# chao1224/MoleculeSDE

Hardware: AMD Instinct MI355X
Metric: molecules/sec pretrain step (SchNet+SDE VE, bs256) (higher is better)
Workload: dtype f32; 1 GPU; PCQM4Mv2-shaped pretrain step: GIN5x300 + SchNet(6x128f,51g,rc10) + EBM_node_dot_prod contrastive + SDEModel2Dto3D_02 VE; fwd+bwd+Adam; molecules_per_gpu=256, global_batch=256, parallelism=dp1

## Files before the change

moleculesde_amd/csrc/linear.hip:

```cpp
#include "msde_common.h"

typedef float f32x16 __attribute__((ext_vector_type(16)));

#define LG_BK 32
#ifndef MSDE_WGRAD_NARROW
#define MSDE_WGRAD_NARROW 7
#endif
#ifndef LG_SKIP_DEAD
#define LG_SKIP_DEAD 1
#endif
#ifndef LG_PRIO
#define LG_PRIO 2
#endif
#ifndef LG_ST
#define LG_ST 1
#endif

__device__ __forceinline__ float4 lg_ldg4(const void* p) {
#if defined(__HIP_DEVICE_COMPILE__)
  typedef float lg_v4f __attribute__((ext_vector_type(4)));
  const lg_v4f v = *(const __attribute__((address_space(1))) lg_v4f*)(p);
  return make_float4(v.x, v.y, v.z, v.w);
#else
  return *reinterpret_cast<const float4*>(p);
#endif
}
__device__ __forceinline__ float lg_ldg1(const float* p) {
#if defined(__HIP_DEVICE_COMPILE__)
  return *(const __attribute__((address_space(1))) float*)(p);
#else
  return *p;
#endif
}

#ifdef LG_PROBE
__device__ unsigned long long lg_probe[8];
#define LG_T(x) __builtin_amdgcn_sched_barrier(0); const unsigned long long x = __builtin_readcyclecounter(); __builtin_amdgcn_sched_barrier(0)
extern "C" int msde_debug_lg_probe(unsigned long long* host8, int reset) {
  if (host8 && hipMemcpyFromSymbol(host8, HIP_SYMBOL(lg_probe), sizeof(lg_probe)) != hipSuccess) return MSDE_EINVAL;
  if (reset) { unsigned long long z[8] = {0}; if (hipMemcpyToSymbol(HIP_SYMBOL(lg_probe), z, sizeof(z)) != hipSuccess) return MSDE_EINVAL; }
  return 0;
}
#else
#define LG_T(x)
#endif

template <int TM, int TN, bool A_KM, bool B_KM, bool VEC, int WGM = 2, int KS = 1>
__device__ __forceinline__ void
gemm_f32_mfma_body(const float* __restrict__ A, const float* __restrict__ B, const float* __restrict__ bias,
                   float* __restrict__ C, float* __restrict__ colsum_ws, int M, int N, int K, int lda, int ldb,
                   int ldc, int k_per_split, const int bid_x, const int bid_y, const int bid_z, float* __restrict__ As,
                   float* __restrict__ Bs, const bool edge_fast = false) {
  constexpr int WGN = KS == 4 ? 1 : 4 / WGM;
  constexpr int BM = 32 * (KS == 4 ? 1 : WGM) * TM, BN = 32 * WGN * TN;
  constexpr int BK = LG_BK * KS;
  static_assert(KS == 1 || (KS == 4 && TM == 1 && TN == 1 && WGM == 1 && A_KM && B_KM), "k-split tiles: 32 x 32, k-major operands");
  static_assert(WGM == 2 || (TM == 1 && TN == 1 && A_KM && B_KM), "side-by-side wave layouts: weight-gradient operands only");
  constexpr int LDA_S = A_KM ? (KS == 4 ? 32 : BM <= 64 ? 64 : (WGM == 2 ? BM + 4 : BM)) : BM + 1;
  constexpr int LDB_S = B_KM ? (KS == 4 ? 32 : BN <= 64 ? 64 : (WGM == 2 ? BN + 4 : BN)) : BN + 1;

  int tid_ = threadIdx.x;
  asm volatile("" : "+v"(tid_));
  const int tid = tid_, lane = tid & 63, wave = tid >> 6;
  const int lcol = lane & 31, lhalf = lane >> 5;
  const int wm = KS == 4 ? 0 : wave / WGN, wn = KS == 4 ? 0 : wave % WGN;
  const int kq = KS == 4 ? wave * LG_BK : 0;
  const int m0 = bid_y * BM, n0 = bid_x * BN;
  const int kb = bid_z * k_per_split;
  const int ke = max(min(K, kb + k_per_split), kb);

  constexpr int NA = BM * BK / 1024, NB = BN * BK / 1024;
  static_assert(NA >= 1 && NB >= 1, "tile too small for 256 threads");
  constexpr int ST = LG_ST;
  float4 rsa[ST][NA], rsb[ST][NB];

  auto ld4 = [&](const float* __restrict__ base, int row, int nrows, int ld, int col, int ncols, bool vec) -> float4 {
    bool rv = row < nrows;
    int rc = rv ? row : 0;
    const float* src = base + (size_t)rc * ld;
    float4 v;
    if (vec) {
      bool cv = col < ncols;
      v = lg_ldg4(src + (cv ? col : 0));
      if (!(rv && cv)) v = make_float4(0.f, 0.f, 0.f, 0.f);
    } else {
      float x0 = lg_ldg1(src + (col < ncols ? col : 0)), x1 = lg_ldg1(src + (col + 1 < ncols ? col + 1 : 0));
      float x2 = lg_ldg1(src + (col + 2 < ncols ? col + 2 : 0)), x3 = lg_ldg1(src + (col + 3 < ncols ? col + 3 : 0));
      v.x = (rv && col < ncols) ? x0 : 0.f;
      v.y = (rv && col + 1 < ncols) ? x1 : 0.f;
      v.z = (rv && col + 2 < ncols) ? x2 : 0.f;
      v.w = (rv && col + 3 < ncols) ? x3 : 0.f;
    }
    return v;
  };

  auto load_tile = [&](float4 (&ra)[NA], float4 (&rb)[NB], int k0) {
#pragma unroll
    for (int p = 0; p < NA; ++p) {
      int idx = p * 256 + tid;
      if (!A_KM) {
        int r = idx >> 3, kq = (idx & 7) * 4;
        ra[p] = ld4(A, m0 + r, M, lda, k0 + kq, ke, VEC);
      } else {
        int kr = idx / (BM / 4), mq = (idx % (BM / 4)) * 4;
        ra[p] = ld4(A, k0 + kr, ke, lda, m0 + mq, M, VEC);
      }
    }
#pragma unroll
    for (int p = 0; p < NB; ++p) {
      int idx = p * 256 + tid;
      if (!B_KM) {
        int r = idx >> 3, kq = (idx & 7) * 4;
        rb[p] = ld4(B, n0 + r, N, ldb, k0 + kq, ke, VEC);
      } else {
        int kr = idx / (BN / 4), nq = (idx % (BN / 4)) * 4;
        rb[p] = ld4(B, k0 + kr, ke, ldb, n0 + nq, N, VEC);
      }
    }
  };

  constexpr bool FAST = A_KM && B_KM && VEC;
  const bool interior = FAST && (edge_fast ? (M >= 4 && N >= 4) : (m0 + BM <= M && n0 + BN <= N));
  unsigned oa[NA], ob[NB];
  if (FAST) {
#pragma unroll
    for (int p = 0; p < NA; ++p) {
      const int idx = p * 256 + tid, kr = idx / (BM / 4), mq = min((idx % (BM / 4)) * 4, M - 4 - m0);
      oa[p] = (unsigned)(((long long)kr * lda + mq) * 4);
    }
#pragma unroll
    for (int p = 0; p < NB; ++p) {
      const int idx = p * 256 + tid, kr = idx / (BN / 4), nq = min((idx % (BN / 4)) * 4, N - 4 - n0);
      ob[p] = (unsigned)(((long long)kr * ldb + nq) * 4);
    }
  }
  auto load_tile_fast = [&](float4 (&ra)[NA], float4 (&rb)[NB], int k0) {
    const char* __restrict__ ab = reinterpret_cast<const char*>(A + (size_t)k0 * lda + m0);
    const char* __restrict__ bb = reinterpret_cast<const char*>(B + (size_t)k0 * ldb + n0);
#pragma unroll
    for (int p = 0; p < NA; ++p) ra[p] = lg_ldg4(ab + oa[p]);
#pragma unroll
    for (int p = 0; p < NB; ++p) rb[p] = lg_ldg4(bb + ob[p]);
  };

  auto store_tile = [&](const float4 (&ra)[NA], const float4 (&rb)[NB]) {
#pragma unroll
    for (int p = 0; p < NA; ++p) {
      int idx = p * 256 + tid;
      if (!A_KM) {
        int r = idx >> 3, kq = (idx & 7) * 4;
        As[(kq + 0) * LDA_S + r] = ra[p].x;
        As[(kq + 1) * LDA_S + r] = ra[p].y;
        As[(kq + 2) * LDA_S + r] = ra[p].z;
        As[(kq + 3) * LDA_S + r] = ra[p].w;
      } else {
        int kr = idx / (BM / 4), mq = (idx % (BM / 4)) * 4;
        *reinterpret_cast<float4*>(&As[kr * LDA_S + mq]) = ra[p];
      }
    }
#pragma unroll
    for (int p = 0; p < NB; ++p) {
      int idx = p * 256 + tid;
      if (!B_KM) {
        int r = idx >> 3, kq = (idx & 7) * 4;
        Bs[(kq + 0) * LDB_S + r] = rb[p].x;
        Bs[(kq + 1) * LDB_S + r] = rb[p].y;
        Bs[(kq + 2) * LDB_S + r] = rb[p].z;
        Bs[(kq + 3) * LDB_S + r] = rb[p].w;
      } else {
        int kr = idx / (BN / 4), nq = (idx % (BN / 4)) * 4;
        *reinterpret_cast<float4*>(&Bs[kr * LDB_S + nq]) = rb[p];
      }
    }
  };

  f32x16 acc[TM][TN];
#pragma unroll
  for (int i = 0; i < TM; ++i)
#pragma unroll
    for (int j = 0; j < TN; ++j)
#pragma unroll
      for (int r = 0; r < 16; ++r) acc[i][j][r] = 0.f;

  float csum = 0.f;

  const bool quadrant_live = !LG_SKIP_DEAD || ((m0 + wm * 32 * TM < M) && (n0 + wn * 32 * TN < N));
  bool sub_live[TM][TN];
#pragma unroll
  for (int i = 0; i < TM; ++i)
#pragma unroll
    for (int j = 0; j < TN; ++j)
      sub_live[i][j] = (m0 + (wm * TM + i) * 32 < M) && (n0 + (wn * TN + j) * 32 < N);
#ifdef LG_PROBE
  unsigned long long pt4 = 0, pacc[6] = {0, 0, 0, 0, 0, 0};
#endif
  auto compute_tile = [&]() {
    if (TM == 1 && TN == 1) {
      if (quadrant_live) {
      float af[LG_BK / 2], bf[LG_BK / 2];
#pragma unroll
      for (int kk = 0; kk < LG_BK / 2; ++kk) {
        af[kk] = As[(kq + 2 * kk + lhalf) * LDA_S + wm * 32 + lcol];
        bf[kk] = Bs[(kq + 2 * kk + lhalf) * LDB_S + wn * 32 + lcol];
      }
      __builtin_amdgcn_sched_barrier(0);
#ifdef LG_PROBE
      pt4 = __builtin_readcyclecounter();
      __builtin_amdgcn_sched_barrier(0);
#endif
      __builtin_amdgcn_s_setprio(LG_PRIO);
#pragma unroll
      for (int kk = 0; kk < LG_BK / 2; ++kk)
        acc[0][0] = __builtin_amdgcn_mfma_f32_32x32x2f32(af[kk], bf[kk], acc[0][0], 0, 0, 0);
      __builtin_amdgcn_s_setprio(0);
      }
    } else {
    __builtin_amdgcn_s_setprio(LG_PRIO);
#pragma unroll
    for (int kk = 0; kk < LG_BK / 2; ++kk) {
      float af[TM], bf[TN];
#pragma unroll
      for (int i = 0; i < TM; ++i) af[i] = As[(2 * kk + lhalf) * LDA_S + (wm * TM + i) * 32 + lcol];
#pragma unroll
      for (int j = 0; j < TN; ++j) bf[j] = Bs[(2 * kk + lhalf) * LDB_S + (wn * TN + j) * 32 + lcol];
#pragma unroll
      for (int i = 0; i < TM; ++i)
#pragma unroll
        for (int j = 0; j < TN; ++j)
          if (!LG_SKIP_DEAD || sub_live[i][j])
            acc[i][j] = __builtin_amdgcn_mfma_f32_32x32x2f32(af[i], bf[j], acc[i][j], 0, 0, 0);
    }
    __builtin_amdgcn_s_setprio(0);
    }
    if (colsum_ws != nullptr && bid_x == 0) {
      if (A_KM && (BM == 64 || WGM != 2)) {
        constexpr int CG = 256 / BM;
        const int c = tid % BM, q = tid / BM;
#pragma unroll
        for (int kr = 0; kr < BK / CG; ++kr) csum += As[(q * (BK / CG) + kr) * LDA_S + c];
      } else if (tid < BM) {
#pragma unroll 8
        for (int kr = 0; kr < LG_BK; ++kr) csum += As[kr * LDA_S + tid];
      }
    }
  };

  const int ntiles = (ke - kb + BK - 1) / BK;
  if (ntiles > 0) {
#pragma unroll
    for (int s = 0; s < ST; ++s) load_tile(rsa[s], rsb[s], kb + s * BK);
    int t = 0;
    if (FAST && interior) {
      const int nfull = (ke - kb) / BK;
      for (; t + 2 * ST <= nfull; t += ST) {
#pragma unroll
        for (int s = 0; s < ST; ++s) {
          LG_T(t0);
          __syncthreads();
          LG_T(t1);
          store_tile(rsa[s], rsb[s]);
          LG_T(t2);
          __syncthreads();
          LG_T(t3);
          load_tile_fast(rsa[s], rsb[s], kb + (t + s + ST) * BK);
          compute_tile();
          LG_T(t5);
#ifdef LG_PROBE
          pacc[0] += t1 - t0; pacc[1] += t2 - t1; pacc[2] += t3 - t2; pacc[3] += pt4 - t3; pacc[4] += t5 - pt4; pacc[5] += 1;
#endif
        }
      }
    }
    for (; t + ST <= ntiles; t += ST) {
#pragma unroll
      for (int s = 0; s < ST; ++s) {
        __syncthreads();
        store_tile(rsa[s], rsb[s]);
        __syncthreads();
        load_tile(rsa[s], rsb[s], kb + (t + s + ST) * BK);
        compute_tile();
      }
    }
    const int rem = ntiles - t;
#pragma unroll
    for (int s = 0; s < ST - 1; ++s) {
      if (s < rem) {
        __syncthreads();
        store_tile(rsa[s], rsb[s]);
        __syncthreads();
        compute_tile();
      }
    }
  }

#ifdef LG_PROBE
  if (tid == 0 && quadrant_live)
    for (int i = 0; i < 6; ++i) atomicAdd(&lg_probe[i], pacc[i]);
#endif
  float* Cz = C + (size_t)bid_z * (size_t)M * ldc;
  if (KS == 4) {
    __syncthreads();
#pragma unroll
    for (int r = 0; r < 16; ++r) As[(wave * 16 + r) * 64 + lane] = acc[0][0][r];
    __syncthreads();
    const int gn = n0 + lcol;
#pragma unroll
    for (int j = 0; j < 4; ++j) {
      const int r = 4 * wave + j;
      const float v = ((As[r * 64 + lane] + As[(16 + r) * 64 + lane]) + As[(32 + r) * 64 + lane]) + As[(48 + r) * 64 + lane];
      const int gm = m0 + (r & 3) + 8 * (r >> 2) + 4 * lhalf;
      if (gm < M && gn < N) Cz[(size_t)gm * ldc + gn] = v;
    }
  } else {
#pragma unroll
  for (int i = 0; i < TM; ++i)
#pragma unroll
    for (int j = 0; j < TN; ++j) {
      int gn = n0 + (wn * TN + j) * 32 + lcol;
      float bv = (bias != nullptr && gn < N) ? bias[gn] : 0.f;
#pragma unroll
      for (int r = 0; r < 16; ++r) {
        int gm = m0 + (wm * TM + i) * 32 + (r & 3) + 8 * (r >> 2) + 4 * lhalf;
        if (gm < M && gn < N) Cz[(size_t)gm * ldc + gn] = acc[i][j][r] + bv;
      }
    }
  }
  if (colsum_ws != nullptr && bid_x == 0) {
    if (A_KM && (BM == 64 || WGM != 2)) {
      constexpr int CG = 256 / BM;
      __syncthreads();
      Bs[tid] = csum;
      __syncthreads();
      if (tid < BM) {
        csum = Bs[tid];
#pragma unroll
        for (int q = 1; q < CG; ++q) csum += Bs[q * BM + tid];
      }
    }
    if (tid < BM && m0 + tid < M) colsum_ws[(size_t)bid_z * M + m0 + tid] = csum;
  }
}

template <int TM, int TN, bool A_KM, bool B_KM, bool VEC>
__global__ void __launch_bounds__(256)
gemm_f32_mfma_kernel(const float* __restrict__ A, const float* __restrict__ B, const float* __restrict__ bias,
                     float* __restrict__ C, float* __restrict__ colsum_ws, int M, int N, int K, int lda, int ldb,
                     int ldc, int k_per_split, const int* __restrict__ Kdev) {
  constexpr int BM = 64 * TM, BN = 64 * TN;
  constexpr int LDA_S = A_KM ? (BM == 64 ? 64 : BM + 4) : BM + 1, LDB_S = B_KM ? (BN == 64 ? 64 : BN + 4) : BN + 1;
  __shared__ __attribute__((aligned(16))) float As[LG_BK * LDA_S];
  __shared__ __attribute__((aligned(16))) float Bs[LG_BK * LDB_S];
  gemm_f32_mfma_body<TM, TN, A_KM, B_KM, VEC>(A, B, bias, C, colsum_ws, M, N, msde_true_rows(K, Kdev), lda, ldb, ldc,
                                              k_per_split, blockIdx.x, blockIdx.y, blockIdx.z, As, Bs);
}

__device__ __forceinline__ void
gemm_grouped_wgrad_body(const long long* __restrict__ probs, const int* __restrict__ prefix, int count, int total,
                          int xcd_order) {
  __shared__ __attribute__((aligned(16))) float lds[8192];
  for (int blk = blockIdx.x; blk < total; blk += gridDim.x) {
    int lo = 0, hi = count;
    while (hi - lo > 1) {
      int mid = (lo + hi) >> 1;
      if (prefix[mid] <= blk) lo = mid; else hi = mid;
    }
    const long long* e = probs + (size_t)lo * MSDE_WGRAD_ROW;
    const float* gY = reinterpret_cast<const float*>(e[0]);
    const float* X = reinterpret_cast<const float*>(e[1]);
    float* slabs = reinterpret_cast<float*>(e[2]);
    float* cs = reinterpret_cast<float*>(e[3]);
    const int M = (int)e[4], N = (int)e[5], K = (int)e[6], kps = (int)e[8], tx = (int)e[9], ty = (int)e[10];
    const int ldg = (int)e[12], ldx = (int)e[13];
    const int Mt = msde_true_rows(M, reinterpret_cast<const int*>(e[14]));
    int local = blk - prefix[lo];
    if (xcd_order) {
      const int np = prefix[lo + 1] - prefix[lo], q = np >> 3, r = np & 7, c = local & 7;
      local = c * q + min(c, r) + (local >> 3);
    }
    const int bx = local % tx, by = (local / tx) % ty, bz = local / (tx * ty);
    const int shape = (int)(e[15] >> 1);
    float* As = lds;
    float* Bs = lds + 4096;
    if ((MSDE_WGRAD_NARROW & 1) && e[11] && shape == 1)
      gemm_f32_mfma_body<1, 1, true, true, true, 1, 1>(gY, X, nullptr, slabs, cs, N, K, Mt, ldg, ldx, K, kps, bx, by, bz, As, Bs, true);
    else if ((MSDE_WGRAD_NARROW & 2) && e[11] && shape == 2)
      gemm_f32_mfma_body<1, 1, true, true, true, 4, 1>(gY, X, nullptr, slabs, cs, N, K, Mt, ldg, ldx, K, kps, bx, by, bz, As, Bs, true);
    else if ((MSDE_WGRAD_NARROW & 4) && e[11] && shape == 3)
      gemm_f32_mfma_body<1, 1, true, true, true, 1, 4>(gY, X, nullptr, slabs, cs, N, K, Mt, ldg, ldx, K, kps, bx, by, bz, As, Bs, true);
    else if (e[11])
      gemm_f32_mfma_body<1, 1, true, true, true>(gY, X, nullptr, slabs, cs, N, K, Mt, ldg, ldx, K, kps, bx, by, bz, As, Bs,
                                                 (e[15] & 1) != 0);
    else
      gemm_f32_mfma_body<1, 1, true, true, false>(gY, X, nullptr, slabs, cs, N, K, Mt, ldg, ldx, K, kps, bx, by, bz, As, Bs);
    __syncthreads();
  }
}

__global__ void __launch_bounds__(256)
gemm_grouped_wgrad_kernel(const long long* __restrict__ probs, const int* __restrict__ prefix, int count, int total,
                          int xcd_order) {
  gemm_grouped_wgrad_body(probs, prefix, count, total, xcd_order);
}
__global__ void __launch_bounds__(256) __attribute__((amdgpu_waves_per_eu(4, 4)))
gemm_grouped_wgrad_occ4_kernel(const long long* __restrict__ probs, const int* __restrict__ prefix, int count, int total,
                               int xcd_order) {
  gemm_grouped_wgrad_body(probs, prefix, count, total, xcd_order);
}

#define RS_LANES 16
__global__ void __launch_bounds__(256)
reduce_slabs_kernel(const float* __restrict__ slabs, int splits, size_t n, float* __restrict__ out,
                    const float* __restrict__ cs, size_t nb, float* __restrict__ outb) {
  __shared__ float part[RS_LANES][16];
  const int ox = threadIdx.x & 15, ly = threadIdx.x >> 4;
  size_t total = n + (cs ? nb : 0);
  for (size_t base = (size_t)blockIdx.x * 16; base < total; base += (size_t)gridDim.x * 16) {
    size_t i = base + ox;
    float acc = 0.f;
    if (i < total) {
      const float* src = i < n ? slabs + i : cs + (i - n);
      size_t stride = i < n ? n : nb;
      for (int z = ly; z < splits; z += RS_LANES) acc += src[(size_t)z * stride];
    }
    part[ly][ox] = acc;
    __syncthreads();
    if (ly == 0 && i < total) {
      float r = part[0][ox];
#pragma unroll
      for (int l = 1; l < RS_LANES; ++l) r += part[l][ox];
      if (i < n) out[i] = r; else outb[i - n] = r;
    }
    __syncthreads();
  }
}

int msde_reduce_slabs(const float* slabs, int splits, size_t n, float* out, const float* cs, size_t nb, float* outb,
                      hipStream_t st) {
  size_t total = n + (cs ? nb : 0);
  int blocks = (int)((total + 15) / 16);
  if (blocks > 4096) blocks = 4096;
  if (blocks < 1) blocks = 1;
  MSDE_LAUNCH(reduce_slabs_kernel, dim3(blocks), dim3(256), 0, st, slabs, splits, n, out, cs, nb, outb);
  MSDE_CHECK_LAUNCH();
  return 0;
}

static inline bool aligned16(const void* p) { return (reinterpret_cast<uintptr_t>(p) & 15) == 0; }

template <int TM, int TN, bool A_KM, bool B_KM>
static void launch_cfg(bool vec, dim3 grid, hipStream_t st, const float* A, const float* B, const float* bias, float* C,
                       float* colsum_ws, int M, int N, int K, int lda, int ldb, int ldc, int k_per_split, const int* kdev) {
  if (vec)
    MSDE_LAUNCH((gemm_f32_mfma_kernel<TM, TN, A_KM, B_KM, true>), grid, dim3(256), 0, st, A, B, bias, C, colsum_ws, M, N,
                K, lda, ldb, ldc, k_per_split, kdev);
  else
    MSDE_LAUNCH((gemm_f32_mfma_kernel<TM, TN, A_KM, B_KM, false>), grid, dim3(256), 0, st, A, B, bias, C, colsum_ws, M,
                N, K, lda, ldb, ldc, k_per_split, kdev);
}

template <bool A_KM, bool B_KM>
static int launch_gemm(const float* A, const float* B, const float* bias, float* C, float* colsum_ws, int M, int N,
                       int K, int lda, int ldb, int ldc, int splits, int k_per_split, bool big, hipStream_t st,
                       const int* kdev = nullptr) {
  bool vec = aligned16(A) && aligned16(B) && (lda % 4 == 0) && (ldb % 4 == 0) && (k_per_split % 4 == 0);
  vec = vec && ((A_KM ? M : K) % 4 == 0) && ((B_KM ? N : K) % 4 == 0);
  int tm, tn;
  if (big) {
    tm = M > 64 ? 2 : 1;
    tn = N > 64 ? 2 : 1;
  } else {
    long t22 = (long)((M + 127) / 128) * ((N + 127) / 128);
    long t21 = (long)((M + 127) / 128) * ((N + 63) / 64);
    if (t22 >= 384) { tm = 2; tn = 2; }
    else if (t21 >= 256) { tm = 2; tn = 1; }
    else { tm = 1; tn = 1; }
  }
  dim3 grid((N + 64 * tn - 1) / (64 * tn), (M + 64 * tm - 1) / (64 * tm), splits);
#define LG_ARGS vec, grid, st, A, B, bias, C, colsum_ws, M, N, K, lda, ldb, ldc, k_per_split, kdev
  if (tm == 2 && tn == 2) launch_cfg<2, 2, A_KM, B_KM>(LG_ARGS);
  else if (tm == 2 && tn == 1) launch_cfg<2, 1, A_KM, B_KM>(LG_ARGS);
  else if (tm == 1 && tn == 2) launch_cfg<1, 2, A_KM, B_KM>(LG_ARGS);
  else launch_cfg<1, 1, A_KM, B_KM>(LG_ARGS);
#undef LG_ARGS
  hipError_t e = hipGetLastError();
  return e == hipSuccess ? 0 : (int)e;
}

__global__ void __launch_bounds__(256) zero_words_kernel(uint32_t* __restrict__ p, size_t n) {
  for (size_t i = (size_t)blockIdx.x * 256 + threadIdx.x; i < n; i += (size_t)gridDim.x * 256) p[i] = 0u;
}
__global__ void __launch_bounds__(256) zero_words4_kernel(uint4* __restrict__ p, size_t n4) {
  for (size_t i = (size_t)blockIdx.x * 256 + threadIdx.x; i < n4; i += (size_t)gridDim.x * 256) p[i] = make_uint4(0u, 0u, 0u, 0u);
}

int msde_zero_words(void* p, size_t n_words, hipStream_t st) {
  if (n_words == 0) return 0;
  if (!p || (reinterpret_cast<uintptr_t>(p) & 3)) return MSDE_EINVAL;
  if ((reinterpret_cast<uintptr_t>(p) & 15) == 0 && n_words % 4 == 0) {
    size_t n4 = n_words / 4, wg = (n4 + 255) / 256;
    MSDE_LAUNCH(zero_words4_kernel, dim3((unsigned)(wg < 4096 ? wg : 4096)), dim3(256), 0, st, reinterpret_cast<uint4*>(p), n4);
  } else {
    size_t wg = (n_words + 255) / 256;
    MSDE_LAUNCH(zero_words_kernel, dim3((unsigned)(wg < 4096 ? wg : 4096)), dim3(256), 0, st, reinterpret_cast<uint32_t*>(p), n_words);
  }
  MSDE_CHECK_LAUNCH();
  return 0;
}

extern "C" int msde_linear_fwd(const float* X, const float* W, const float* bias, int M, int N, int K, float* Y,
                               void* stream) {
  if (M < 0 || N <= 0 || K <= 0 || !X || !W || !Y) return MSDE_EINVAL;
  if (M == 0) return 0;
  return launch_gemm<false, false>(X, W, bias, Y, nullptr, M, N, K, K, K, N, 1, (K + 31) / 32 * 32, false,
                                    as_stream(stream));
}

extern "C" int msde_linear_bwd_x(const float* gY, const float* W, int M, int N, int K, float* gX, void* stream) {
  if (M < 0 || N <= 0 || K <= 0 || !gY || !W || !gX) return MSDE_EINVAL;
  if (M == 0) return 0;
  return launch_gemm<false, true>(gY, W, nullptr, gX, nullptr, M, K, N, N, K, K, 1, (N + 31) / 32 * 32, false,
                                   as_stream(stream));
}

static inline bool wgrad_big(int M, int N, int K) {
  return false;
}
static inline void wgrad_split_for(int M, int N, int K, int target, int* splits, int* k_per_split);
static inline void wgrad_split(int M, int N, int K, int* splits, int* k_per_split) {
  const int target = 512;
  wgrad_split_for(M, N, K, target, splits, k_per_split);
}
#ifndef MSDE_WGRAD_TARGET
#define MSDE_WGRAD_TARGET 64
#endif
#ifndef MSDE_WGRAD_MIN_ROWS
#define MSDE_WGRAD_MIN_ROWS 256
#endif
#ifndef MSDE_WGRAD_TARGET_KS
#define MSDE_WGRAD_TARGET_KS 64
#endif
static inline void wgrad_split_batched(int M, int N, int K, int* splits, int* k_per_split) {
  const int target = (N <= 32 && K <= 32 && (MSDE_WGRAD_NARROW & 4)) ? MSDE_WGRAD_TARGET_KS : MSDE_WGRAD_TARGET;
  wgrad_split_for(M, N, K, target, splits, k_per_split);
}
static inline void wgrad_split_for(int M, int N, int K, int target, int* splits, int* k_per_split) {
  bool big = wgrad_big(M, N, K);
  int tw_n = (big && N > 64) ? 128 : 64, tw_k = (big && K > 64) ? 128 : 64;
  long tiles = (long)((N + tw_n - 1) / tw_n) * ((K + tw_k - 1) / tw_k);
  long want = (target + tiles - 1) / tiles;
  long maxs = (M + MSDE_WGRAD_MIN_ROWS - 1) / MSDE_WGRAD_MIN_ROWS;
  if (maxs < 1) maxs = 1;
  if (want > maxs) want = maxs;
  if (want > 512) want = 512;
  if (want < 1) want = 1;
  int kps = (int)(((M + want - 1) / want + LG_BK - 1) / LG_BK * LG_BK);
  if (kps < LG_BK) kps = LG_BK;
  *k_per_split = kps;
  *splits = M > 0 ? (M + kps - 1) / kps : 1;
}

static inline bool wgrad_group_plan(int M, int N, int K, int* splits, int* k_per_split) {
  wgrad_split_batched(M, N, K, splits, k_per_split);
  return false;
}

extern "C" long long msde_linear_bwd_w_workspace_bytes(int M, int N, int K) {
  int splits, kps;
  wgrad_split(M, N, K, &splits, &kps);
  return (long long)splits * ((long long)N * K + N) * (long long)sizeof(float);
}

__global__ void __launch_bounds__(256)
reduce_slabs_multi_kernel(const long long* __restrict__ rows, const int* __restrict__ prefix, int count) {
  __shared__ float4 part[256];
  int lo = 0, hi = count;
  while (hi - lo > 1) {
    int mid = (lo + hi) >> 1;
    if (prefix[mid] <= (int)blockIdx.x) lo = mid; else hi = mid;
  }
  const long long* e = rows + (size_t)lo * 8;
  const float* slabs = reinterpret_cast<const float*>(e[0]);
  const int splits = (int)e[1];
  const size_t n = (size_t)e[2];
  float* out = reinterpret_cast<float*>(e[3]);
  const size_t row_len = (size_t)e[4], slab_ld = (size_t)e[5], out_ld = (size_t)e[6], sstride = (size_t)e[7];
  const int LY = splits >= MSDE_REDUCE_LONG ? 16 : 4, OXN = 256 / LY;
  const int ox = threadIdx.x % OXN, ly = threadIdx.x / OXN;
  const size_t i = (size_t)(blockIdx.x - prefix[lo]) * (4 * OXN) + 4 * ox;
  const bool flat = row_len == n;
  const bool vec = (n % 4 == 0) && ((reinterpret_cast<uintptr_t>(slabs) | reinterpret_cast<uintptr_t>(out)) & 15) == 0 &&
                   (flat ? sstride % 4 == 0 : ((row_len | slab_ld | out_ld | sstride) % 4 == 0));
  size_t so[4], oo[4];
#pragma unroll
  for (int q = 0; q < 4; ++q) {
    const size_t j = i + q;
    if (flat) { so[q] = j; oo[q] = j; }
    else { const size_t r = j / row_len, c = j - r * row_len; so[q] = r * slab_ld + c; oo[q] = r * out_ld + c; }
  }
  float4 acc = make_float4(0.f, 0.f, 0.f, 0.f);
  if (i < n) {
    if (vec) {
      const float* base = slabs + so[0];
      int z = ly;
      for (; z + 3 * LY < splits; z += 4 * LY) {
        float4 a = *reinterpret_cast<const float4*>(base + (size_t)z * sstride);
        float4 b = *reinterpret_cast<const float4*>(base + (size_t)(z + LY) * sstride);
        float4 c = *reinterpret_cast<const float4*>(base + (size_t)(z + 2 * LY) * sstride);
        float4 d = *reinterpret_cast<const float4*>(base + (size_t)(z + 3 * LY) * sstride);
        acc = vadd(vadd(vadd(vadd(acc, a), b), c), d);
      }
      for (; z < splits; z += LY) acc = vadd(acc, *reinterpret_cast<const float4*>(base + (size_t)z * sstride));
    } else {
      const bool h1 = i + 1 < n, h2 = i + 2 < n, h3 = i + 3 < n;
      int z = ly;
      for (; z + 3 * LY < splits; z += 4 * LY) {
        const float* p0 = slabs + (size_t)z * sstride;
        const float* p1 = slabs + (size_t)(z + LY) * sstride;
        const float* p2 = slabs + (size_t)(z + 2 * LY) * sstride;
        const float* p3 = slabs + (size_t)(z + 3 * LY) * sstride;
        const float a0 = p0[so[0]], a1 = p1[so[0]], a2 = p2[so[0]], a3 = p3[so[0]];
        const float b0 = h1 ? p0[so[1]] : 0.f, b1 = h1 ? p1[so[1]] : 0.f, b2 = h1 ? p2[so[1]] : 0.f, b3 = h1 ? p3[so[1]] : 0.f;
        const float c0 = h2 ? p0[so[2]] : 0.f, c1 = h2 ? p1[so[2]] : 0.f, c2 = h2 ? p2[so[2]] : 0.f, c3 = h2 ? p3[so[2]] : 0.f;
        const float d0 = h3 ? p0[so[3]] : 0.f, d1 = h3 ? p1[so[3]] : 0.f, d2 = h3 ? p2[so[3]] : 0.f, d3 = h3 ? p3[so[3]] : 0.f;
        acc.x = (((acc.x + a0) + a1) + a2) + a3;
        acc.y = (((acc.y + b0) + b1) + b2) + b3;
        acc.z = (((acc.z + c0) + c1) + c2) + c3;
        acc.w = (((acc.w + d0) + d1) + d2) + d3;
      }
      for (; z < splits; z += LY) {
        const float* p = slabs + (size_t)z * sstride;
        acc.x += p[so[0]];
        if (h1) acc.y += p[so[1]];
        if (h2) acc.z += p[so[2]];
        if (h3) acc.w += p[so[3]];
      }
    }
  }
  part[ly * OXN + ox] = acc;
  __syncthreads();
  if (ly == 0 && i < n) {
    float4 r = part[ox];
    for (int q = 1; q < LY; ++q) r = vadd(r, part[q * OXN + ox]);
    if (vec) {
      *reinterpret_cast<float4*>(out + oo[0]) = r;
    } else {
      out[oo[0]] = r.x;
      if (i + 1 < n) out[oo[1]] = r.y;
      if (i + 2 < n) out[oo[2]] = r.z;
      if (i + 3 < n) out[oo[3]] = r.w;
    }
  }
}

extern "C" long long msde_reduce_slabs_chunks(long long n, int splits) {
  const long long per = splits >= MSDE_REDUCE_LONG ? 64 : 256;
  return (n + per - 1) / per;
}

extern "C" int msde_reduce_slabs_multi(const long long* rows, const int* prefix, int count, int total_chunks,
                                       void* stream) {
  if (count < 0 || total_chunks < 0 || (count > 0 && (!rows || !prefix))) return MSDE_EINVAL;
  if (count == 0 || total_chunks == 0) return 0;
  MSDE_LAUNCH(reduce_slabs_multi_kernel, dim3(total_chunks), dim3(256), 0, as_stream(stream), rows, prefix, count);
  MSDE_CHECK_LAUNCH();
  return 0;
}

extern "C" int msde_linear_bwd_w_describe(const float* gY, const float* X, int M, int N, int K, int want_bias,
                                          float* slabs, const int* rows_dev, long long* row) {
  return msde_linear_bwd_w_describe_ld(gY, N, X, K, M, N, K, want_bias, slabs, rows_dev, row);
}

extern "C" int msde_linear_bwd_w_describe_ld(const float* gY, int ldg, const float* X, int ldx, int M, int N, int K,
                                             int want_bias, float* slabs, const int* rows_dev, long long* row) {
  if (M <= 0 || N <= 0 || K <= 0 || !gY || !X || !slabs || !row || ldg < N || ldx < K) return MSDE_EINVAL;
  if (wgrad_big(M, N, K)) return MSDE_EUNSUP;
  bool vec = aligned16(gY) && aligned16(X) && (N % 4 == 0) && (K % 4 == 0) && (ldg % 4 == 0) && (ldx % 4 == 0);
  int splits, kps;
  wgrad_group_plan(M, N, K, &splits, &kps);
  vec = vec && (kps % 4 == 0);
  int shape = 0;
  if (vec) {
    if (N <= 32 && K <= 32) shape = (MSDE_WGRAD_NARROW & 4) ? 3 : 0;
    else if (N <= 32 && K > 64) shape = (MSDE_WGRAD_NARROW & 1) ? 1 : 0;
    else if (K <= 32 && N > 64) shape = (MSDE_WGRAD_NARROW & 2) ? 2 : 0;
  }
  const int bm = (shape == 1 || shape == 3) ? 32 : shape == 2 ? 128 : 64, bn = (shape == 2 || shape == 3) ? 32 : shape == 1 ? 128 : 64;
  int tx = (K + bn - 1) / bn, ty = (N + bm - 1) / bm;
  const int relax = 0;
  row[12] = ldg; row[13] = ldx; row[14] = reinterpret_cast<long long>(rows_dev); row[15] = relax | (shape << 1);
  row[0] = reinterpret_cast<long long>(gY);
  row[1] = reinterpret_cast<long long>(X);
  row[2] = reinterpret_cast<long long>(slabs);
  row[3] = want_bias ? reinterpret_cast<long long>(slabs + (size_t)splits * N * K) : 0;
  row[4] = M; row[5] = N; row[6] = K; row[7] = splits; row[8] = kps; row[9] = tx; row[10] = ty; row[11] = vec ? 1 : 0;
  return tx * ty * splits;
}

extern "C" int msde_linear_bwd_w_grouped_ex(const long long* probs, const int* prefix, int count, int total_blocks,
                                            int max_workgroups, void* stream) {
  if (count < 0 || total_blocks < 0 || (count > 0 && (!probs || !prefix))) return MSDE_EINVAL;
  if (count == 0 || total_blocks == 0) return 0;
  const int xcd = 1;
  const int grid = max_workgroups > 0 && max_workgroups < total_blocks ? max_workgroups : total_blocks;
  const int occ4 = 0;
  if (occ4)
    MSDE_LAUNCH(gemm_grouped_wgrad_occ4_kernel, dim3(grid), dim3(256), 0, as_stream(stream), probs, prefix, count, total_blocks,
                grid == total_blocks ? xcd : 0);
  else
    MSDE_LAUNCH(gemm_grouped_wgrad_kernel, dim3(grid), dim3(256), 0, as_stream(stream), probs, prefix, count, total_blocks,
                grid == total_blocks ? xcd : 0);
  MSDE_CHECK_LAUNCH();
  return 0;
}

extern "C" int msde_linear_bwd_w_grouped(const long long* probs, const int* prefix, int count, int total_blocks,
                                         void* stream) {
  return msde_linear_bwd_w_grouped_ex(probs, prefix, count, total_blocks, 0, stream);
}

extern "C" int msde_linear_bwd_w_splits(int M, int N, int K) {
  int splits, kps;
  wgrad_group_plan(M, N, K, &splits, &kps);
  return splits;
}

extern "C" int msde_linear_bwd_w_partial(const float* gY, const float* X, int M, int N, int K, int want_bias,
                                         float* slabs, const int* rows_dev, void* stream) {
  if (M <= 0 || N <= 0 || K <= 0 || !gY || !X || !slabs) return MSDE_EINVAL;
  int splits, k_per_split;
  wgrad_group_plan(M, N, K, &splits, &k_per_split);
  float* cs = want_bias ? slabs + (size_t)splits * N * K : nullptr;
  return launch_gemm<true, true>(gY, X, nullptr, slabs, cs, N, K, M, N, K, K, splits, k_per_split, wgrad_big(M, N, K),
                                 as_stream(stream), rows_dev);
}

extern "C" int msde_linear_bwd_w(const float* gY, const float* X, int M, int N, int K, float* gW, float* gb,
                                 float* workspace, const int* rows_dev, void* stream) {
  if (M < 0 || N <= 0 || K <= 0 || !gY || !X || !gW || !workspace) return MSDE_EINVAL;
  hipStream_t st = as_stream(stream);
  int splits, k_per_split;
  wgrad_split(M, N, K, &splits, &k_per_split);
  float* slabs = workspace;
  float* cs = gb ? workspace + (size_t)splits * N * K : nullptr;
  if (M == 0) {
    int e = msde_zero_words(gW, (size_t)N * K, st);
    if (e == 0 && gb) e = msde_zero_words(gb, (size_t)N, st);
    return e;
  }
  if (splits == 1)
    return launch_gemm<true, true>(gY, X, nullptr, gW, gb, N, K, M, N, K, K, 1, k_per_split, wgrad_big(M, N, K), st, rows_dev);
  int rc = launch_gemm<true, true>(gY, X, nullptr, slabs, cs, N, K, M, N, K, K, splits, k_per_split, wgrad_big(M, N, K), st, rows_dev);
  if (rc != 0) return rc;
  return msde_reduce_slabs(slabs, splits, (size_t)N * K, gW, cs, (size_t)N, gb, st);
}
```

Baseline: 100,600 molecules/s.

## Add direct global-to-LDS multi-buffered pipeline for grouped weight-gradient GEMM

Adds a new weight-gradient GEMM body that loads A and B tiles straight into LDS with buffer_load ... lds instructions, using a 3-stage ring buffer and vmcnt-based waits. This overlaps global loads with MFMA compute and skips the register round trip. The grouped wgrad kernel now sends shape 0, 1 and 2 vectorized problems to this path. LDS allocation grows to a larger aligned buffer, which may lower occupancy, and the inline asm depends on buffer-resource and M0 semantics being correct.

```diff
diff --git a/moleculesde_amd/csrc/linear.hip b/moleculesde_amd/csrc/linear.hip
--- a/moleculesde_amd/csrc/linear.hip
+++ b/moleculesde_amd/csrc/linear.hip
@@ -1,4 +1,5 @@
 #include "msde_common.h"
+#include <type_traits>
 
 typedef float f32x16 __attribute__((ext_vector_type(16)));
 
@@ -354,10 +355,173 @@
                                               k_per_split, blockIdx.x, blockIdx.y, blockIdx.z, As, Bs);
 }
 
+#ifndef LG_GLDS
+#define LG_GLDS 1
+#endif
+#ifndef LG_GBK
+#define LG_GBK 32
+#endif
+#ifndef LG_NBUF
+#define LG_NBUF 3
+#endif
+#define LG_RING_FLOATS (LG_NBUF * LG_GBK * 128)
+#define LG_LDS_FLOATS (LG_RING_FLOATS > 10240 ? LG_RING_FLOATS : 10240)
+#define LG_NBUF_NARROW (LG_LDS_FLOATS / 5120 > 3 ? 3 : LG_LDS_FLOATS / 5120)
+
+typedef int lg_i32x4 __attribute__((ext_vector_type(4)));
+__device__ __forceinline__ lg_i32x4 lg_rsrc(const void* p, unsigned bytes) {
+  const unsigned long long a = (unsigned long long)p;
+  lg_i32x4 r;
+  r.x = (int)(unsigned)(a & 0xFFFFFFFFull);
+  r.y = (int)(unsigned)((a >> 32) & 0xFFFFull);
+  r.z = (int)bytes;
+  r.w = 0x00020000;
+  return r;
+}
+__device__ __forceinline__ void lg_glds(unsigned voff, lg_i32x4 rsrc, unsigned lds_addr) {
+  asm volatile("s_mov_b32 m0, %2\n\ts_nop 0\n\tbuffer_load_dwordx4 %0, %1, 0 offen lds"
+               :
+               : "v"(voff), "s"(rsrc), "s"(lds_addr)
+               : "memory");
+}
+template <int N> __device__ __forceinline__ void lg_wait_vm() { asm volatile("s_waitcnt vmcnt(%0)" ::"n"(N > 63 ? 63 : N) : "memory"); }
+__device__ __forceinline__ void lg_barrier() {
+  __builtin_amdgcn_sched_barrier(0);
+  asm volatile("s_waitcnt lgkmcnt(0)\n\ts_barrier" ::: "memory");
+  __builtin_amdgcn_sched_barrier(0);
+}
+
+template <int WGM, int BK, int NB>
+__device__ __forceinline__ void
+wgrad_glds_body(const float* __restrict__ A, const float* __restrict__ B, float* __restrict__ C, float* __restrict__ colsum_ws,
+                int M, int N, int K, int lda, int ldb, int ldc, int k_per_split, const int bid_x, const int bid_y, const int bid_z,
+                float* __restrict__ lds) {
+  constexpr int WGN = 4 / WGM;
+  constexpr int BM = 32 * WGM, BN = 32 * WGN;
+  constexpr int PA = BK * BM / 256, PB = BK * BN / 256;
+  constexpr int PW = (PA + PB) / 4;
+  constexpr int STF = BK * (BM + BN);
+  static_assert(PA % 4 == 0 && PB % 4 == 0 && BK % 32 == 0 && NB >= 2 && NB <= 4, "geometry");
+  int tid_ = threadIdx.x;
+  asm volatile("" : "+v"(tid_));
+  const int tid = tid_, lane = tid & 63;
+  const int wave = __builtin_amdgcn_readfirstlane(tid >> 6);
+  const int lcol = lane & 31, lhalf = lane >> 5;
+  const int wm = wave / WGN, wn = wave % WGN;
+  const int m0 = bid_y * BM, n0 = bid_x * BN;
+  const int kb = bid_z * k_per_split;
+  const int ke = __builtin_amdgcn_readfirstlane(max(min(K, kb + k_per_split), kb));
+  const int ntiles = (ke - kb + BK - 1) / BK;
+
+  unsigned vo[PW];
+#pragma unroll
+  for (int i = 0; i < PW; ++i) {
+    const int p = 4 * i + wave;
+    if (4 * i < PA) {
+      const int r = p * (256 / BM) + lane / (BM / 4), c = 4 * (lane % (BM / 4));
+      vo[i] = (unsigned)(r * lda + c) * 4u;
+    } else {
+      const int q = p - PA, r = q * (256 / BN) + lane / (BN / 4), c = 4 * (lane % (BN / 4));
+      vo[i] = (unsigned)(r * ldb + c) * 4u;
+    }
+  }
+  const unsigned lds0 = (unsigned)(size_t)(__attribute__((address_space(3))) float*)lds;
+  const int colsA = min(BM, M - m0), colsB = min(BN, N - n0);
+  auto issue = [&](int t, int s) __attribute__((always_inline)) {
+    const int k0 = kb + t * BK, rv = min(BK, ke - k0);
+    const lg_i32x4 ra = lg_rsrc(A + (size_t)k0 * lda + m0, (unsigned)(((rv - 1) * lda + colsA) * 4));
+    const lg_i32x4 rb = lg_rsrc(B + (size_t)k0 * ldb + n0, (unsigned)(((rv - 1) * ldb + colsB) * 4));
+    const unsigned sb = lds0 + (unsigned)(s * STF * 4);
+#pragma unroll
+    for (int i = 0; i < PW; ++i) {
+      const unsigned la = sb + (unsigned)(4 * i + wave) * 1024u;
+      if (4 * i < PA) lg_glds(vo[i], ra, la);
+      else lg_glds(vo[i], rb, la);
+    }
+  };
+
+  f32x16 acc;
+#pragma unroll
+  for (int r = 0; r < 16; ++r) acc[r] = 0.f;
+  float csum = 0.f;
+  const bool quadrant_live = !LG_SKIP_DEAD || ((m0 + wm * 32 < M) && (n0 + wn * 32 < N));
+  const bool want_cs = colsum_ws != nullptr && bid_x == 0;
+  constexpr int CG = 256 / BM;
+
+  auto ktile = [&](auto live_, auto last_, int t, int stage) __attribute__((always_inline)) {
+    constexpr bool LIVE = decltype(live_)::value, LAST = decltype(last_)::value;
+    if (LAST) lg_wait_vm<0>();
+    else if (NB >= 4 && t + 2 < ntiles) lg_wait_vm<2 * PW>();
+    else if (NB >= 3) lg_wait_vm<PW>();
+    else lg_wait_vm<0>();
+    lg_barrier();
+    if (!LAST && t + NB - 1 < ntiles) issue(t + NB - 1, stage == 0 ? NB - 1 : stage - 1);
+    const float* As = lds + stage * STF;
+    const float* Bs = As + BK * BM;
+    const int k0 = kb + t * BK;
+#pragma unroll
+    for (int sb = 0; sb < BK / 32; ++sb) {
+      if (LAST && sb > 0 && k0 + 32 * sb >= ke) break;
+      if (LIVE) {
+        float af[16], bf[16];
+#pragma unroll
+        for (int kk = 0; kk < 16; ++kk) {
+          af[kk] = As[(32 * sb + 2 * kk + lhalf) * BM + wm * 32 + lcol];
+          bf[kk] = Bs[(32 * sb + 2 * kk + lhalf) * BN + wn * 32 + lcol];
+        }
+        __builtin_amdgcn_sched_barrier(0);
+        __builtin_amdgcn_s_setprio(LG_PRIO);
+#pragma unroll
+        for (int kk = 0; kk < 16; ++kk) acc = __builtin_amdgcn_mfma_f32_32x32x2f32(af[kk], bf[kk], acc, 0, 0, 0);
+        __builtin_amdgcn_s_setprio(0);
+      }
+      if (want_cs) {
+        const int c = tid % BM, q = tid / BM;
+#pragma unroll
+        for (int kr = 0; kr < 32 / CG; ++kr) csum += As[(32 * sb + q * (32 / CG) + kr) * BM + c];
+      }
+    }
+  };
+  auto run = [&](auto live_) __attribute__((always_inline)) {
+#pragma unroll
+    for (int s = 0; s < NB - 1; ++s)
+      if (s < ntiles) issue(s, s);
+    int stage = 0;
+    for (int t = 0; t + 1 < ntiles; ++t) {
+      ktile(live_, std::false_type{}, t, stage);
+      stage = stage + 1 == NB ? 0 : stage + 1;
+    }
+    if (ntiles > 0) ktile(live_, std::true_type{}, ntiles - 1, stage);
+  };
+  if (quadrant_live) run(std::true_type{});
+  else run(std::false_type{});
+
+  float* Cz = C + (size_t)bid_z * (size_t)M * ldc;
+  {
+    const int gn = n0 + wn * 32 + lcol;
+#pragma unroll
+    for (int r = 0; r < 16; ++r) {
+      const int gm = m0 + wm * 32 + (r & 3) + 8 * (r >> 2) + 4 * lhalf;
+      if (gm < M && gn < N) Cz[(size_t)gm * ldc + gn] = acc[r];
+    }
+  }
+  __syncthreads();
+  if (want_cs) {
+    lds[tid] = csum;
+    __syncthreads();
+    if (tid < BM) {
+      csum = lds[tid];
+#pragma unroll
+      for (int q = 1; q < CG; ++q) csum += lds[q * BM + tid];
+      if (m0 + tid < M) colsum_ws[(size_t)bid_z * M + m0 + tid] = csum;
+    }
+  }
+}
+
 __device__ __forceinline__ void
 gemm_grouped_wgrad_body(const long long* __restrict__ probs, const int* __restrict__ prefix, int count, int total,
                           int xcd_order) {
-  __shared__ __attribute__((aligned(16))) float lds[8192];
+  __shared__ __attribute__((aligned(1024))) float lds[LG_LDS_FLOATS];
   for (int blk = blockIdx.x; blk < total; blk += gridDim.x) {
     int lo = 0, hi = count;
     while (hi - lo > 1) {
@@ -381,7 +545,13 @@
     const int shape = (int)(e[15] >> 1);
     float* As = lds;
     float* Bs = lds + 4096;
-    if ((MSDE_WGRAD_NARROW & 1) && e[11] && shape == 1)
+    if (LG_GLDS && e[11] && shape == 0)
+      wgrad_glds_body<2, LG_GBK, LG_NBUF>(gY, X, slabs, cs, N, K, Mt, ldg, ldx, K, kps, bx, by, bz, lds);
+    else if (LG_GLDS && (MSDE_WGRAD_NARROW & 1) && e[11] && shape == 1)
+      wgrad_glds_body<1, 32, LG_NBUF_NARROW>(gY, X, slabs, cs, N, K, Mt, ldg, ldx, K, kps, bx, by, bz, lds);
+    else if (LG_GLDS && (MSDE_WGRAD_NARROW & 2) && e[11] && shape == 2)
+      wgrad_glds_body<4, 32, LG_NBUF_NARROW>(gY, X, slabs, cs, N, K, Mt, ldg, ldx, K, kps, bx, by, bz, lds);
+    else if ((MSDE_WGRAD_NARROW & 1) && e[11] && shape == 1)
       gemm_f32_mfma_body<1, 1, true, true, true, 1, 1>(gY, X, nullptr, slabs, cs, N, K, Mt, ldg, ldx, K, kps, bx, by, bz, As, Bs, true);
     else if ((MSDE_WGRAD_NARROW & 2) && e[11] && shape == 2)
       gemm_f32_mfma_body<1, 1, true, true, true, 4, 1>(gY, X, nullptr, slabs, cs, N, K, Mt, ldg, ldx, K, kps, bx, by, bz, As, Bs, true);
```

After: 101,800 molecules/s (median of 6 runs). 1.01x the previous value.
